# mattmireles/Mamba-ASR

Measured on AMD Instinct MI355X. Metric: encoder audio-frames/sec (ConMamba-large, L=4000), higher is better.
Workload: dtype bf16; 1 GPU; conmamba_large_ctc: encoder forward, 64 utterances x 4000 frames (1000 scan steps) per GPU, random-init weights; global_batch=64, frames_per_utterance=4000, parallelism=utterance shards x1 (no collective in forward), launch=hipGraph replay, streams=2 (join)

## Files before the change

### include/conmamba_hip.h

```cpp
#ifndef CONMAMBA_HIP_H
#define CONMAMBA_HIP_H

#include <stdint.h>

#ifdef __cplusplus
extern "C" {
#endif

#define CM_ABI_VERSION 12

#define CM_OK            0
#define CM_EINVAL       (-1)
#define CM_EUNSUPPORTED (-2)
#define CM_EALIGN       (-3)

typedef enum { CM_F32 = 0, CM_BF16 = 1, CM_F16 = 2 } cm_dtype;

#define CM_SCAN_CHUNK 64

int         cm_abi_version(void);
const char *cm_last_error(void);
int         cm_scan_num_chunks(int seqlen);
#ifdef CM_ABLATE
int         cm_debug_set(int ablation);
// ... 528 lines not shown
    float       *dweight;
    float       *dbias;
    int64_t x_bs, x_ds, y_bs, y_ds, dy_bs, dy_ds, dx_bs, dx_ds;
    void *stream;
} cm_dwconv1d_args;

int cm_dwconv1d_fwd(const cm_dwconv1d_args *args);
int cm_dwconv1d_bwd(const cm_dwconv1d_args *args);

typedef struct cm_dwconv_cl_args {
    int32_t batch, dim, seqlen, ksize, pad_left;
    int32_t io_dtype;
    const void  *x;
    const float *weight;
    const float *bias;
    void        *y;
    const void  *dy;
    void        *dx;
    float       *dweight;
    float       *dbias;
    float       *partial;
    int64_t x_bs, x_ts, y_bs, y_ts, dy_bs, dy_ts, dx_bs, dx_ts;
    void *stream;
    int32_t overwrite;
    int32_t reserved0;
} cm_dwconv_cl_args;

int64_t cm_dwconv_cl_workspace_floats(int32_t batch, int32_t seqlen, int32_t dim);
int cm_dwconv_cl_fwd(const cm_dwconv_cl_args *args);
int cm_dwconv_cl_bwd(const cm_dwconv_cl_args *args);

typedef struct cm_layernorm_args {
    int64_t rows;
    int32_t dim;
    int32_t x_dtype, y_dtype;
    float   eps;
    const void  *x;
    const float *gamma, *beta;
    void  *y;
    float *mean, *rstd;
    const void *dy;
    void  *dx;
    float *dgamma, *dbeta;
    float *workspace;
    void  *stream;
    const float *dres;
    int32_t act;
    float   act_slope;
    const float *chan_mask;
    int32_t mask_rows, mask_c;
} cm_layernorm_args;

int64_t cm_layernorm_bwd_workspace_floats(int64_t rows, int32_t dim);
int cm_layernorm_fwd(const cm_layernorm_args *args);
int cm_layernorm_bwd(const cm_layernorm_args *args);

typedef struct cm_ln_pw_glu_args {
    int32_t rows, dim;
    const float *x;
    const void  *y;
    const float *ln_g, *ln_b;
    const void  *w;
    const float *bias;
    float *x_out;
    void  *out;
    float alpha, eps;
    void *stream;
} cm_ln_pw_glu_args;

int cm_ln_pw_glu(const cm_ln_pw_glu_args *args);

typedef struct cm_ln_pw_glu_mix_args {
    int32_t rows, dim;
    const float *x;
    const float *ln_g, *ln_b;
    const void  *w;
    const float *bias;
    float *x_out;
    void  *out;
    float alpha, eps;
    void *stream;
    const void *ycat;
    const void *proj_w;
    int32_t proj_k;
} cm_ln_pw_glu_mix_args;

int cm_ln_pw_glu_mix(const cm_ln_pw_glu_mix_args *args);

typedef struct cm_cnn_block1_args {
    int32_t batch, T, F, C;
    int32_t io_dtype;
    int32_t pad_out;
    const float *feats;
    const float *weight;
    const float *bias;
    const float *ln_g, *ln_b;
    float eps, slope;
    void *out;
    void *stream;
} cm_cnn_block1_args;

int cm_cnn_block1(const cm_cnn_block1_args *args);

typedef struct cm_cnn_block2_args {
    int32_t batch, T_in, F_in, C_in, C_out;
    int32_t pad_;
    const void  *in;
    const void  *weight;
    const float *bias;
    const float *ln_g, *ln_b;
    float eps, slope;
    void *out;
    void *stream;
} cm_cnn_block2_args;

int cm_cnn_block2(const cm_cnn_block2_args *args);

typedef struct cm_cnn_front_args {
    int32_t batch, T, F, C1, C2;
    int32_t pad_;
    const float *feats;
    const float *w1, *b1, *ln1_g, *ln1_b;
    const void  *w2;
    const float *b2, *ln2_g, *ln2_b;
    float eps1, eps2, slope;
    int32_t pad2_;
    void *out;
    void *stream;
} cm_cnn_front_args;

int cm_cnn_front(const cm_cnn_front_args *args);

typedef struct cm_gemm_args {
    int32_t M, N, K;
    int32_t epilogue;
    const void  *A;  int64_t lda;
    const void  *W;  int64_t ldw;
    const float *bias;
    void        *out; int64_t ldo;
    float       *x;
    float alpha, eps1, eps2;
    int32_t pad_;
    const float *g1, *b1, *g2, *b2;
    void *stream;
} cm_gemm_args;

int cm_gemm_bf16(const cm_gemm_args *args);

int cm_ffn_pack_weights(const void *w , int32_t rows, int32_t cols,
                        void *out , void *stream);

typedef struct cm_ffn_args {
    int32_t rows, dim, hidden;
    int32_t h_dtype;
    const float *x;
    const void  *addend;
    const float *pre_g, *pre_b;
    const void  *w1;
    const float *b1;
    const void  *w2;
    const float *b2;
    const float *n1_g, *n1_b;
    const float *n2_g, *n2_b;
    float       *x_out;
    void        *h_out;
    float add_scale, alpha, pre_eps, n1_eps, n2_eps;
    int32_t proj_dim;
// ... 86 lines not shown
```

### mamba_asr_amd/csrc/ln_pw_glu.hip

```cpp
#include "cm_common.h"


namespace {

typedef __attribute__((ext_vector_type(8))) __bf16 bf16x8;
typedef __attribute__((ext_vector_type(2))) __bf16 bf16x2;
typedef __attribute__((ext_vector_type(4))) float f32x4;
typedef __attribute__((ext_vector_type(2))) float f32x2;
typedef __attribute__((ext_vector_type(4))) unsigned int u32x4;

constexpr int D = 256;
constexpr int TOK = 64;
constexpr int XS = 264;

__device__ __forceinline__ void lds_barrier() { asm volatile("s_waitcnt lgkmcnt(0)\n\ts_barrier" ::: "memory"); }
__device__ __forceinline__ uint32_t pack2(float a, float b) {
    return __builtin_bit_cast(uint32_t, __builtin_convertvector(f32x2{a, b}, bf16x2));
}

constexpr int CK = 128;
constexpr int STAGE = TOK * CK * 2;
static_assert(2 * STAGE <= TOK * XS * 2, "the two ycat stages must fit the token tile they overlay");

struct mix_extra {
    const void *ycat;
    const void *proj_w;
    int32_t proj_k;
};

__device__ __forceinline__ u32x4 raw_rsrc(const void *base, uint32_t bytes) {
    const uint64_t a = reinterpret_cast<uint64_t>(base);
    return u32x4{(uint32_t)a, (uint32_t)(a >> 32) & 0xffffu, bytes, 0x00020000u};
}
__device__ __forceinline__ void dma16(const u32x4 rsrc, uint32_t lds_addr, int voff) {
    uint32_t keep;
    asm volatile("s_mov_b32 %0, m0\n\ts_mov_b32 m0, %1\n\ts_nop 0\n\tbuffer_load_dwordx4 %2, %3, 0 offen lds\n\ts_mov_b32 m0, %0"
                 : "=&s"(keep)
                 : "s"(lds_addr), "v"(voff), "s"(rsrc)
                 : "memory");
}

template <int OCC, int PF, bool MIX>
__global__ __launch_bounds__(256, OCC) void ln_pw_glu_kernel(const cm_ln_pw_glu_args p, const mix_extra mx) {
    __shared__ __attribute__((aligned(16))) uint16_t xn[TOK * XS];
    const int tid = threadIdx.x, lane = tid & 63;
    const int wave = __builtin_amdgcn_readfirstlane(tid >> 6);
    const int l15 = lane & 15, lq = lane >> 4;
    const int t0 = blockIdx.x * TOK, M = p.rows;
    const uint16_t *yv = reinterpret_cast<const uint16_t *>(p.y);

    const __amdgpu_buffer_rsrc_t wr = __builtin_amdgcn_make_buffer_rsrc(const_cast<void *>(p.w), 0, 2 * D * D * 2, 0x00020000);
    const int vl = lane * 16;
    auto wload = [&](int ps, int s, bf16x8(&dst)[2]) {
        const int half = s >> 3, ks = s & 7;
#pragma unroll
        for (int mb = 0; mb < 2; ++mb)
            dst[mb] = __builtin_bit_cast(bf16x8, __builtin_amdgcn_raw_buffer_load_b128(
                                                     wr, vl, (((half * D + wave * 64) / 16 + 2 * ps + mb) * (D / 32) + ks) * 1024, 0));
    };
    bf16x8 wq[PF][2];
    if constexpr (MIX) {
        static_assert(PF == 2, "the projection phase's ring indexing assumes two steps in flight");
        const int K = mx.proj_k, kt = K / 32, nch = K / CK, nstep = 2 * kt;
        const __amdgpu_buffer_rsrc_t pr = __builtin_amdgcn_make_buffer_rsrc(const_cast<void *>(mx.proj_w), 0, D * K * 2, 0x00020000);
        auto pload = [&](int g, bf16x8(&dst)[2]) {
            g = min(g, nstep - 1);
            const int ks = g >> 1, mp = g & 1;
#pragma unroll
            for (int mb = 0; mb < 2; ++mb)
                dst[mb] = __builtin_bit_cast(bf16x8, __builtin_amdgcn_raw_buffer_load_b128(pr, vl, ((wave * 4 + mp * 2 + mb) * kt + ks) * 1024, 0));
        };
        const int vrows = min(TOK, M - t0);
        const u32x4 yr = raw_rsrc(reinterpret_cast<const unsigned char *>(mx.ycat) + (int64_t)t0 * K * 2, (uint32_t)(vrows * K * 2));
        const uint32_t lds0 = (uint32_t)reinterpret_cast<uintptr_t>(&xn[0]);
        int go[4];
#pragma unroll
        for (int i = 0; i < 4; ++i) {
            const int row = 4 * (4 * wave + i) + lq;
            go[i] = row * K * 2 + 16 * (l15 ^ (((row & 3) << 2) | ((row >> 2) & 3)));
        }
        auto request = [&](int c) {
#pragma unroll
            for (int i = 0; i < 4; ++i) dma16(yr, lds0 + (uint32_t)((c & 1) * STAGE + (4 * wave + i) * 1024), go[i] + c * (CK * 2));
        };
        request(0);
#pragma unroll
        for (int s = 0; s < PF; ++s) pload(s, wq[s]);
        f32x4 acc[4][4];
#pragma unroll
        for (int mb = 0; mb < 4; ++mb)
#pragma unroll
            for (int nb = 0; nb < 4; ++nb) acc[mb][nb] = f32x4{0.f, 0.f, 0.f, 0.f};
        const unsigned char *xb = reinterpret_cast<const unsigned char *>(xn);
        const int yrow = l15 * (CK * 2), yswz = ((l15 & 3) << 2) | (l15 >> 2);
        auto read_y = [&](int st, int kk, bf16x8(&bf)[4]) {
            const int off = st * STAGE + yrow + 16 * ((kk * 4 + lq) ^ yswz);
#pragma unroll
            for (int nb = 0; nb < 4; ++nb) bf[nb] = *reinterpret_cast<const bf16x8 *>(xb + off + nb * 16 * (CK * 2));
        };
        for (int c = 0; c < nch; ++c) {
            asm volatile("s_waitcnt vmcnt(0)" ::: "memory");
            lds_barrier();
            if (c + 1 < nch) request(c + 1);
            const int st = c & 1;
            bf16x8 bf[4];
#pragma unroll
            for (int s = 0; s < 8; ++s) {
                const int kk = s >> 1, mp = s & 1;
                if (mp == 0) read_y(st, kk, bf);
#pragma unroll
                for (int mb = 0; mb < 2; ++mb)
#pragma unroll
                    for (int nb = 0; nb < 4; ++nb)
                        acc[mp * 2 + mb][nb] = __builtin_amdgcn_mfma_f32_16x16x32_bf16(wq[s % PF][mb], bf[nb], acc[mp * 2 + mb][nb], 0, 0, 0);
                pload(c * 8 + s + PF, wq[s % PF]);
                __builtin_amdgcn_sched_barrier(0);
            }
        }
        lds_barrier();
#pragma unroll
        for (int mb = 0; mb < 4; ++mb)
#pragma unroll
            for (int nb = 0; nb < 4; ++nb)
                *reinterpret_cast<uint2 *>(xn + (nb * 16 + l15) * XS + wave * 64 + mb * 16 + lq * 4) =
                    uint2{pack2(acc[mb][nb][0], acc[mb][nb][1]), pack2(acc[mb][nb][2], acc[mb][nb][3])};
    }
    if constexpr (MIX) lds_barrier();
    else {
#pragma unroll
        for (int s = 0; s < PF; ++s) wload(0, s, wq[s]);
    }

    {
        float4 v[4][4];
#pragma unroll
        for (int rd = 0; rd < 4; ++rd) {
            const int tok = min(t0 + wave * 16 + rd * 4 + lq, M - 1);
#pragma unroll
            for (int i = 0; i < 4; ++i) {
                const int col = (l15 + 16 * i) * 4;
                float4 x4 = *reinterpret_cast<const float4 *>(p.x + (int64_t)tok * D + col);
                if (MIX || yv) {
                    const uint2 a = MIX ? *reinterpret_cast<const uint2 *>(xn + (wave * 16 + rd * 4 + lq) * XS + col)
                                        : *reinterpret_cast<const uint2 *>(yv + (int64_t)tok * D + col);
                    x4.x = fmaf(p.alpha, cm_bf16_lo(a.x), x4.x);
                    x4.y = fmaf(p.alpha, cm_bf16_hi(a.x), x4.y);
                    x4.z = fmaf(p.alpha, cm_bf16_lo(a.y), x4.z);
                    x4.w = fmaf(p.alpha, cm_bf16_hi(a.y), x4.w);
                }
                v[rd][i] = x4;
            }
        }
#pragma unroll
        for (int rd = 0; rd < 4; ++rd) {
            const int tok = t0 + wave * 16 + rd * 4 + lq;
            if (p.x_out && tok < M) {
#pragma unroll
                for (int i = 0; i < 4; ++i) *reinterpret_cast<float4 *>(p.x_out + (int64_t)tok * D + (l15 + 16 * i) * 4) = v[rd][i];
            }
            float s = 0.f;
#pragma unroll
            for (int i = 0; i < 4; ++i) s += (v[rd][i].x + v[rd][i].y) + (v[rd][i].z + v[rd][i].w);
            const float mean = cm_group_sum<16>(s) * (1.f / D);
            float q = 0.f;
#pragma unroll
            for (int i = 0; i < 4; ++i) {
                v[rd][i].x -= mean; v[rd][i].y -= mean; v[rd][i].z -= mean; v[rd][i].w -= mean;
                q = fmaf(v[rd][i].x, v[rd][i].x, fmaf(v[rd][i].y, v[rd][i].y, fmaf(v[rd][i].z, v[rd][i].z, fmaf(v[rd][i].w, v[rd][i].w, q))));
            }
            const float rstd = rsqrtf(cm_group_sum<16>(q) * (1.f / D) + p.eps);
            uint16_t *dst = xn + (wave * 16 + rd * 4 + lq) * XS;
#pragma unroll
            for (int i = 0; i < 4; ++i) {
                const int col = (l15 + 16 * i) * 4;
                const float4 g = *reinterpret_cast<const float4 *>(p.ln_g + col);
                const float4 b = *reinterpret_cast<const float4 *>(p.ln_b + col);
                uint2 pk;
                pk.x = pack2(fmaf(v[rd][i].x * rstd, g.x, b.x), fmaf(v[rd][i].y * rstd, g.y, b.y));
                pk.y = pack2(fmaf(v[rd][i].z * rstd, g.z, b.z), fmaf(v[rd][i].w * rstd, g.w, b.w));
                *reinterpret_cast<uint2 *>(dst + col) = pk;
            }
        }
    }
    if constexpr (MIX) {
#pragma unroll
        for (int s = 0; s < PF; ++s) wload(0, s, wq[s]);
    }
    lds_barrier();

    const uint16_t *xfrag = xn + l15 * XS + lq * 8;
    auto read_frags = [&](int ks, bf16x8(&bf)[4]) {
#pragma unroll
        for (int nb = 0; nb < 4; ++nb) bf[nb] = *reinterpret_cast<const bf16x8 *>(xfrag + nb * 16 * XS + ks * 32);
    };
    uint16_t *out = reinterpret_cast<uint16_t *>(p.out);
    uint2 held[2][4];
#pragma unroll
    for (int ps = 0; ps < 2; ++ps) {
        f32x4 acc[2][2][4];
#pragma unroll
        for (int h = 0; h < 2; ++h)
#pragma unroll
            for (int mb = 0; mb < 2; ++mb)
#pragma unroll
                for (int nb = 0; nb < 4; ++nb) acc[h][mb][nb] = f32x4{0.f, 0.f, 0.f, 0.f};
        bf16x8 bfa[4], bfb[4];
        read_frags(0, bfa);
#pragma unroll
        for (int s = 0; s < 16; ++s) {
            bf16x8(&cur)[4] = (s & 1) ? bfb : bfa;
            bf16x8(&nxt)[4] = (s & 1) ? bfa : bfb;
            if (s + 1 < 16) read_frags((s + 1) & 7, nxt);
#pragma unroll
            for (int mb = 0; mb < 2; ++mb)
#pragma unroll
                for (int nb = 0; nb < 4; ++nb)
                    acc[s >> 3][mb][nb] = __builtin_amdgcn_mfma_f32_16x16x32_bf16(wq[s % PF][mb], cur[nb], acc[s >> 3][mb][nb], 0, 0, 0);
            if (s + PF < 16) wload(ps, s + PF, wq[s % PF]);
            else if (ps == 0) wload(1, s + PF - 16, wq[s % PF]);
            __builtin_amdgcn_sched_barrier(0);
        }
        const int f0 = wave * 64 + ps * 32 + lq * 4;
#pragma unroll
        for (int mb = 0; mb < 2; ++mb) {
            const float4 ba = *reinterpret_cast<const float4 *>(p.bias + f0 + mb * 16);
            const float4 bg = *reinterpret_cast<const float4 *>(p.bias + D + f0 + mb * 16);
#pragma unroll
            for (int nb = 0; nb < 4; ++nb) {
                const float o0 = (acc[0][mb][nb][0] + ba.x) * cm_sigmoid(acc[1][mb][nb][0] + bg.x);
                const float o1 = (acc[0][mb][nb][1] + ba.y) * cm_sigmoid(acc[1][mb][nb][1] + bg.y);
                const float o2 = (acc[0][mb][nb][2] + ba.z) * cm_sigmoid(acc[1][mb][nb][2] + bg.z);
                const float o3 = (acc[0][mb][nb][3] + ba.w) * cm_sigmoid(acc[1][mb][nb][3] + bg.w);
                if (ps == 0) held[mb][nb] = uint2{pack2(o0, o1), pack2(o2, o3)};
                else {
                    if (mb == 0 && nb == 0) lds_barrier();
                    *reinterpret_cast<uint2 *>(xn + (nb * 16 + l15) * XS + f0 + mb * 16) = uint2{pack2(o0, o1), pack2(o2, o3)};
                    *reinterpret_cast<uint2 *>(xn + (nb * 16 + l15) * XS + f0 - 32 + mb * 16) = held[mb][nb];
                }
            }
        }
    }
    lds_barrier();
#pragma unroll
    for (int i = 0; i < TOK * 32 / 256; ++i) {
        const int idx = tid + 256 * i, row = idx >> 5, chunk = idx & 31;
        const uint4 v = *reinterpret_cast<const uint4 *>(xn + row * XS + chunk * 8);
        if (t0 + row < M) *reinterpret_cast<uint4 *>(out + (int64_t)(t0 + row) * D + chunk * 8) = v;
    }
}

}

int cm_ln_pw_glu144_launch(const cm_ln_pw_glu_args &a);

extern "C" int cm_ln_pw_glu(const cm_ln_pw_glu_args *args) {
    CM_REQUIRE(args != nullptr, CM_EINVAL, "ln_pw_glu: args is NULL");
    const cm_ln_pw_glu_args &a = *args;
    CM_REQUIRE(a.rows > 0 && a.x && a.ln_g && a.ln_b && a.w && a.bias && a.out, CM_EINVAL, "ln_pw_glu: bad sizes or NULL tensor");
    CM_REQUIRE(a.dim == D || a.dim == 144, CM_EUNSUPPORTED, "ln_pw_glu: d_model must be 256 or 144 (got %d)", a.dim);
    CM_REQUIRE(cm_aligned(a.x, 16) && cm_aligned(a.ln_g, 16) && cm_aligned(a.ln_b, 16) && cm_aligned(a.w, 16) && cm_aligned(a.bias, 16) &&
                   cm_aligned(a.out, 16) && (!a.y || cm_aligned(a.y, 8)) && (!a.x_out || cm_aligned(a.x_out, 16)),
               CM_EALIGN, "ln_pw_glu: tensors must be 16-byte aligned (y / out 8)");
    if (a.dim != D) return cm_ln_pw_glu144_launch(a);
    const dim3 grid((a.rows + TOK - 1) / TOK);
    hipStream_t st = reinterpret_cast<hipStream_t>(a.stream);
#ifdef CM_ABLATE
    if (cm_debug_get() == 41) {
        hipLaunchKernelGGL((ln_pw_glu_kernel<3, 4, false>), grid, dim3(256), 0, st, a, mix_extra{});
        return cm_launch_status("cm_ln_pw_glu");
    }
#endif
    hipLaunchKernelGGL((ln_pw_glu_kernel<4, 2, false>), grid, dim3(256), 0, st, a, mix_extra{});
    return cm_launch_status("cm_ln_pw_glu");
}

extern "C" int cm_ln_pw_glu_mix(const cm_ln_pw_glu_mix_args *args) {
    CM_REQUIRE(args != nullptr, CM_EINVAL, "ln_pw_glu_mix: args is NULL");
    const cm_ln_pw_glu_mix_args &m = *args;
    CM_REQUIRE(m.rows > 0 && m.x && m.ln_g && m.ln_b && m.w && m.bias && m.out && m.ycat && m.proj_w, CM_EINVAL,
               "ln_pw_glu_mix: bad sizes or NULL tensor");
    CM_REQUIRE(m.dim == D, CM_EUNSUPPORTED, "ln_pw_glu_mix: d_model must be 256 (got %d)", m.dim);
    CM_REQUIRE(m.proj_k >= CK && m.proj_k % CK == 0 && m.proj_k <= 8192, CM_EUNSUPPORTED,
               "ln_pw_glu_mix: proj_k must be a multiple of 128, at most 8192 (got %d)", m.proj_k);
    CM_REQUIRE(cm_aligned(m.x, 16) && cm_aligned(m.ln_g, 16) && cm_aligned(m.ln_b, 16) && cm_aligned(m.w, 16) && cm_aligned(m.bias, 16) &&
                   cm_aligned(m.out, 16) && cm_aligned(m.ycat, 16) && cm_aligned(m.proj_w, 16) && (!m.x_out || cm_aligned(m.x_out, 16)),
               CM_EALIGN, "ln_pw_glu_mix: tensors must be 16-byte aligned");
    const auto overlap = [](const void *a, int64_t na, const void *b, int64_t nb) {
        const uintptr_t pa = reinterpret_cast<uintptr_t>(a), pb = reinterpret_cast<uintptr_t>(b);
        return a && b && pa < pb + (uintptr_t)nb && pb < pa + (uintptr_t)na;
    };
    const int64_t nx = (int64_t)m.rows * D * 4, no = (int64_t)m.rows * D * 2, ny = (int64_t)m.rows * m.proj_k * 2;
    CM_REQUIRE(!overlap(m.out, no, m.x, nx) && !overlap(m.out, no, m.ycat, ny) && !overlap(m.out, no, m.x_out, nx) &&
                   !overlap(m.x_out, nx, m.ycat, ny) && (m.x_out == m.x || !overlap(m.x_out, nx, m.x, nx)),
               CM_EALIGN, "ln_pw_glu_mix: out / x_out overlap an input (only x_out == x is allowed)");
    cm_ln_pw_glu_args a{};
    a.rows = m.rows, a.dim = m.dim, a.x = m.x, a.y = nullptr, a.ln_g = m.ln_g, a.ln_b = m.ln_b, a.w = m.w, a.bias = m.bias;
    a.x_out = m.x_out, a.out = m.out, a.alpha = m.alpha, a.eps = m.eps, a.stream = m.stream;
    const mix_extra mx{m.ycat, m.proj_w, m.proj_k};
    hipLaunchKernelGGL((ln_pw_glu_kernel<4, 2, true>), dim3((a.rows + TOK - 1) / TOK), dim3(256), 0, reinterpret_cast<hipStream_t>(a.stream), a, mx);
    return cm_launch_status("cm_ln_pw_glu_mix");
}
```

### mamba_asr_amd/fused.py

```python
from __future__ import annotations

import os
from typing import Optional

import torch
import torch.nn.functional as F

from . import ops, weight_cache


class _LayerCache:

    def __init__(self, layer, dtype):
        self.dtype = dtype
        c = lambda t: t.detach().to(dtype).contiguous()
        f = lambda t: None if t is None else t.detach().float().contiguous()
        ffn = lambda m: dict(ln=(f(m[0].weight), f(m[0].bias), m[0].eps), w1=c(m[1].ffn[0].weight), b1=c(m[1].ffn[0].bias),
                             w2=c(m[1].ffn[3].weight), b2=c(m[1].ffn[3].bias), b1f=f(m[1].ffn[0].bias),
                             b2f=f(m[1].ffn[3].bias))
        self.ffn1, self.ffn2 = ffn(layer.ffn_module1), ffn(layer.ffn_module2)
        D = self.ffn1["w1"].shape[1]
        wide = D == 256
        kp = ops._kpad(D)
        d144 = D == 144 and USE_FUSED_D144 and ops.FFN_LAYOUT == 16
        if ops.ffn_supported(D, self.ffn1["w1"].shape[0], dtype) and self.ffn1["w1"].is_cuda and (wide or d144):
            for q in (self.ffn1, self.ffn2):
                q["w1p"] = ops.PackedWeight(q["w1"], ops.FFN_LAYOUT, pad=(q["w1"].shape[0], kp))
                q["w2p"] = ops.PackedWeight(q["w2"], ops.FFN_LAYOUT, pad=(kp, q["w2"].shape[1]))
                if ops.SMALL_FFN_ROWS > 0 and wide:
                    q["w1s"], q["w2s"] = (q["w1p"], q["w2p"]) if ops.FFN_LAYOUT == 32 else (ops.PackedWeight(q["w1"], 32), ops.PackedWeight(q["w2"], 32))
        self.norm1 = (f(layer.norm1.norm.weight), f(layer.norm1.norm.bias), layer.norm1.norm.eps)
        self.norm2 = (f(layer.norm2.norm.weight), f(layer.norm2.norm.bias), layer.norm2.norm.eps)
        m = layer.mamba
        self.d_inner, self.dt_rank, self.d_state = m.d_inner, m.dt_rank, m.d_state
        self.in_proj = c(m.in_proj.weight)
        self.in_packed = None
        if (USE_FFN_INPROJ and dtype == torch.bfloat16 and self.in_proj.is_cuda and self.in_proj.shape[1] == D and (wide or d144)
                and self.in_proj.shape[0] % (256 if wide else 64) == 0 and self.in_proj.shape[0] <= 4096 and m.in_proj.bias is None):
            self.in_packed = ops.PackedWeight(self.in_proj, ops.FFN_LAYOUT, pad=(self.in_proj.shape[0], kp))
            if ops.SMALL_FFN_ROWS > 0 and wide:
                self.in_packed_s = self.in_packed if ops.FFN_LAYOUT == 32 else ops.PackedWeight(self.in_proj, 32)
        self.in_bias = None if m.in_proj.bias is None else c(m.in_proj.bias)
        self.uni = not hasattr(m, "conv1d_b")
        sfxs = ("",) if self.uni else ("", "_b")
        if self.uni:
            self.out_cat = c(m.out_proj.weight)
        else:
            half = 0.5 if m.if_devide_out else 1.0
            self.out_cat = c(torch.cat([m.out_proj.weight, m.out_proj.weight], dim=1) * half)
        self.out_bias = None if m.out_proj.bias is None else c(m.out_proj.bias)
        self.gamma = None if getattr(m, "init_layer_scale", None) is None else f(m.gamma)
        self.dirs = []
        for sfx in sfxs:
            conv, xp, dtp = getattr(m, "conv1d" + sfx), getattr(m, "x_proj" + sfx), getattr(m, "dt_proj" + sfx)
            A_log = getattr(m, "A_b_log" if sfx else "A_log")
            self.dirs.append(dict(conv_w=f(conv.weight).reshape(m.d_inner, -1), conv_b=f(conv.bias), x_proj=c(xp.weight),
                                  dt_proj=c(dtp.weight), dt_proj_f32=c(dtp.weight).float().contiguous(), dt_bias=f(dtp.bias), A=(-torch.exp(A_log.detach().float())).contiguous(),
                                  D=f(getattr(m, "D_b" if sfx else "D"))))
        cm = layer.convolution_module
        xps = [getattr(m, "x_proj" + sfx) for sfx in sfxs]
        self.x_proj_bd = torch.block_diag(*[xp.weight.detach().to(dtype) for xp in xps])
        R, N = self.dt_rank, self.d_state
        self.rows_mode = (R <= 16 or (R <= 32 and dtype == torch.bfloat16)) and N == 16 and m.d_inner % 8 == 0
        if self.rows_mode:
            pad = ops.rows_dt_pad(R)
            self.row_width = pad + 32
            rows = [ops.xproj_rows(xp.weight, R, pad, dtype) for xp in xps]
            self.x_proj_rows = torch.block_diag(*rows)
            self.wx_packed = None
            if dtype == torch.bfloat16 and m.d_inner % 32 == 0 and m.d_inner <= 2048 and rows[0].is_cuda and m.d_conv == 4:
                self.wx_packed = [ops.PackedWeight(r) for r in rows]
            for d_, dtp in zip(self.dirs, [getattr(m, "dt_proj" + sfx) for sfx in sfxs]):
                d_["dt_w16"] = ops.pad_dt_weight(dtp.weight.detach().to(dtype))
        self.cm_ln = (f(cm.layer_norm.weight), f(cm.layer_norm.bias), cm.layer_norm.eps)
        self.pw_w, self.pw_b = c(cm.bottleneck[0].weight.squeeze(-1)), c(cm.bottleneck[0].bias)
        self.pw_bf, self.lin_bf = f(cm.bottleneck[0].bias), f(cm.after_conv[2].bias)
        self.pw_packed = None
        if dtype == torch.bfloat16 and self.pw_w.is_cuda and tuple(self.pw_w.shape) == (2 * D, D) and (wide or d144) and self.pw_bf is not None:
            self.pw_packed = ops.PackedWeight(self.pw_w, pad=(2 * D, kp))
        self.out_packed = None
        if (self.pw_packed is not None and self.out_cat.is_cuda and self.out_cat.shape[0] == 256 and self.out_cat.shape[1] % 128 == 0
                and self.out_cat.shape[1] <= 8192 and self.out_bias is None and self.gamma is None):
            self.out_packed = ops.PackedWeight(self.out_cat)
        self.in_bias_f = None if m.in_proj.bias is None else f(m.in_proj.bias)
        self.out_bias_f = None if m.out_proj.bias is None else f(m.out_proj.bias)
        self.dw_w, self.dw_b = f(cm.conv.weight), f(cm.conv.bias)
        self.dw_wt = self.dw_w.reshape(self.dw_w.shape[0], -1).t().contiguous()
        self.cm_ln2 = (f(cm.after_conv[0].weight), f(cm.after_conv[0].bias), cm.after_conv[0].eps)
        self.lin_w, self.lin_b = c(cm.after_conv[2].weight), c(cm.after_conv[2].bias)
        self.lin_packed = None
        if USE_DWCONV_LIN and dtype == torch.bfloat16 and self.lin_w.is_cuda and tuple(self.lin_w.shape) == (256, 256) and self.lin_bf is not None:
            self.lin_packed = ops.PackedWeight(self.lin_w)
        self.kernel_size, self.causal = cm.kernel_size, bool(cm.causal)

    @property
    def ffn_native(self) -> bool:
        return "w1p" in self.ffn1 and self.ffn2["w1"].shape[0] == self.ffn1["w1"].shape[0]

    @property
    def all_native(self) -> bool:
        return (self.ffn_native and self.rows_mode and self.wx_packed is not None and self.pw_packed is not None
                and self.in_bias is None and self.out_bias is None and self.gamma is None)


def _params_key(dtype, *modules):
    return (dtype,) + tuple((p._version, p.data_ptr()) for m in modules for p in m.parameters())


_LAYER = weight_cache.Kind("_cm_fused_cache", graphs_read=False, build=_LayerCache)


def _cache(layer, dtype) -> _LayerCache:
    return _LAYER.lookup(layer, _params_key(dtype, layer), dtype)


def supports(layer) -> bool:
    from .modules.mamba.bimamba import Mamba as BiMamba, UniMamba
    cm = layer.convolution_module
    act_ok = isinstance(cm.after_conv[1], torch.nn.GELU) and isinstance(layer.ffn_module1[1].ffn[1], torch.nn.GELU)
    mixer_ok = isinstance(layer.mamba, UniMamba) if cm.causal else isinstance(layer.mamba, BiMamba)
    return (mixer_ok and cm.kernel_size == 31 and cm.dilation == 1 and act_ok
            and layer.mamba.d_state == 16 and layer.mamba.d_conv == 4)


def _ffn(x, y_in, p, dtype):
    if dtype == torch.bfloat16:
        h = torch._addmm_activation(p["b1"], y_in, p["w1"].t(), use_gelu=True)
    else:
        h = F.gelu(torch.addmm(p["b1"], y_in, p["w1"].t()))
    return torch.addmm(p["b2"], h, p["w2"].t())


USE_FUSED_D144 = os.environ.get("CM_FUSED_D144", "1") == "1"


USE_FFN_INPROJ = os.environ.get("CM_FFN_INPROJ", "1") == "1"


USE_DWCONV_LIN = os.environ.get("CM_DWCONV_LIN", "1") == "1"


USE_SCAN_ROWS = os.environ.get("CM_SCAN_ROWS", "1") == "1"


USE_CONV_XPROJ = os.environ.get("CM_CONV_XPROJ", "1") == "1"


def _scan_dirs(c: _LayerCache, ucat, ycat, batch, seqlen, xdbl=None):
    E, R, N, nd = c.d_inner, c.dt_rank, c.d_state, len(c.dirs)
    rows, P = batch * seqlen, c.dt_rank + 2 * c.d_state
    if c.rows_mode and (USE_SCAN_ROWS or xdbl is not None):
        if xdbl is None:
            xdbl = (ucat.view(rows, nd * E) @ c.x_proj_rows.t()).view(batch, seqlen, nd * c.row_width)
        RW = c.row_width
        return [dict(u=ucat[:, :, i * E:(i + 1) * E], A=d["A"], D=d["D"], delta_bias=d["dt_bias"], dt_weight=d["dt_w16"],
                     xdbl=xdbl[:, :, RW * i:RW * (i + 1)], out=ycat[:, :, i * E:(i + 1) * E], reverse=bool(i))
                for i, d in enumerate(c.dirs)]
    xdblT = c.x_proj_bd @ ucat.view(rows, nd * E).t()
    feat = ops.alloc_bc(nd * P, batch, seqlen, ucat.device)
    feat.view(nd * P, rows).copy_(xdblT)
    dirs = []
    for i, d in enumerate(c.dirs):
        f = feat[i * P:(i + 1) * P]
        dd = dict(u=ucat[:, :, i * E:(i + 1) * E], A=d["A"], B=f[R:R + N], C=f[R + N:], D=d["D"],
                  delta_bias=d["dt_bias"], out=ycat[:, :, i * E:(i + 1) * E], reverse=bool(i))
        if R <= 16:
            dd.update(dt_low=f[:R], dt_weight=d["dt_proj_f32"])
        else:
            dd["delta"] = (xdblT[i * P:i * P + R].t() @ d["dt_proj"].t()).view(batch, seqlen, E)
        dirs.append(dd)
    return dirs


USE_MIXER_TAIL = os.environ.get("CM_MIXER_TAIL", "1") == "1"


def _out_proj(c: _LayerCache, ycat):
    y = ycat @ c.out_cat.t()
    if c.out_bias is not None:
        y = y + c.out_bias
    if c.gamma is not None:
        y = y * c.gamma.to(y.dtype)
    return y


def mixer_tail(c: _LayerCache, x, ycat):
    if USE_MIXER_TAIL and c.out_packed is not None:
        return ops.ln_pw_glu(x, None, 1.0, c.cm_ln, c.pw_packed, c.pw_bf, ycat=ycat, out_w=c.out_packed)
    return ops.ln_pw_glu(x, _out_proj(c, ycat), 1.0, c.cm_ln, c.pw_packed, c.pw_bf)


def _in_proj(c: _LayerCache, h, out=None):
    xz = torch.mm(h, c.in_proj.t(), out=out)
    return xz if c.in_bias is None else xz.add_(c.in_bias)


def _conv_forms_xdbl(c: _LayerCache) -> bool:
    return USE_CONV_XPROJ and USE_SCAN_ROWS and c.rows_mode and c.wx_packed is not None and c.dtype == torch.bfloat16


def _conv(c: _LayerCache, xz, ucat, xdbl=None, xproj=True, hist=None):
    E = c.d_inner
    if c.uni:
        w0 = (c.dirs[0]["conv_w"], c.dirs[0]["conv_b"])
        if xproj and _conv_forms_xdbl(c):
            x_hist, x_hist_out = hist or (None, None)
            return ops.conv_xproj_uni(xz[:, :, :E], *w0, c.wx_packed[0], out=ucat, xdbl=xdbl, x_hist=x_hist, x_hist_out=x_hist_out)
        assert hist is None
        ops.conv_cl_fwd(xz[:, :, :E], *w0, silu=True, out_f=ucat)
        return None
    w = (c.dirs[0]["conv_w"], c.dirs[0]["conv_b"], c.dirs[1]["conv_w"], c.dirs[1]["conv_b"])
    if xproj and _conv_forms_xdbl(c):
        return ops.conv_xproj(xz[:, :, :E], *w, c.wx_packed[0], c.wx_packed[1], out_f=ucat[:, :, :E], out_b=ucat[:, :, E:], xdbl=xdbl)
    ops.conv_cl_fwd(xz[:, :, :E], *w, True, out_f=ucat[:, :, :E], out_b=ucat[:, :, E:])
    return None


def _scan(c: _LayerCache, xz, ucat, ycat, xdbl, batch, seqlen, state=None):
    dirs = _scan_dirs(c, ucat, ycat, batch, seqlen, xdbl)
    if state is None:
        ops.scan_cl_fwd(dirs, z=xz[:, :, c.d_inner:], delta_softplus=True)
        return
    if len(dirs) != 1 or "xdbl" not in dirs[0]:
        raise NotImplementedError("streaming needs the row-group scan (dt_rank <= 16, or <= 32 in bf16) of a unidirectional mixer")
    ops.scan_cl_fwd([dict(dirs[0], h0=state, h_last=state)], z=xz[:, :, c.d_inner:], delta_softplus=True, time_chunks=1)


def bimamba_fused(c: _LayerCache, h, batch, seqlen):
    xz = _in_proj(c, h).view(batch, seqlen, -1)
    ucat = torch.empty((batch, seqlen, len(c.dirs) * c.d_inner), dtype=xz.dtype, device=xz.device)
    ycat = torch.empty_like(ucat)
    _scan(c, xz, ucat, ycat, _conv(c, xz, ucat), batch, seqlen)
    return _out_proj(c, ycat.view(batch * seqlen, -1))


USE_FUSED_FFN = os.environ.get("CM_FUSED_FFN", "1") == "1"


USE_LN_PW_GLU = os.environ.get("CM_LN_PW_GLU", "1") == "1"


def _ffn_call(x, f, **kw):
    return ops.ffn_fused(x, f["ln"], f["w1p"], f["b1f"], f["w2p"], f["b2f"], alpha=0.5, **kw)


def _ffn_images(c: _LayerCache, small: bool):
    if not (small and "w1s" in c.ffn1):
        return c.ffn1, c.ffn2, c.in_packed
    return (dict(c.ffn1, w1p=c.ffn1["w1s"], w2p=c.ffn1["w2s"]), dict(c.ffn2, w1p=c.ffn2["w1s"], w2p=c.ffn2["w2s"]),
            getattr(c, "in_packed_s", None))


def _head(c: _LayerCache, x, xz, ucat, xdbl=None, small=False, hist=None):
    f1, _, inp = _ffn_images(c, small)
    if c.in_packed is not None:
        _ffn_call(x, f1, norm2=c.norm1, proj_w=inp, proj_out=xz.view(x.shape[0], -1))
    else:
        _in_proj(c, _ffn_call(x, f1, norm2=c.norm1)[1], out=xz.view(x.shape[0], -1))
    return _conv(c, xz, ucat, xdbl, hist=hist)


def _ffn2(c: _LayerCache, x, addend, final_ln=None, f2=None):
    return _ffn_call(x, f2 or c.ffn2, addend=addend, norm1=c.norm2, norm2=final_ln, want_h=final_ln is not None,
                     h_dtype=torch.float32)[1]


def _tail(c: _LayerCache, x, ycat, batch, seqlen, final_ln=None, small=False, hist=None):
    D = x.shape[-1]
    dw = (c.dw_w, c.dw_b, c.cm_ln2[0], c.cm_ln2[1], c.cm_ln2[2])
    kw = dict(causal=True, hist=hist[0], hist_out=hist[1]) if hist is not None else dict(causal=c.causal)
    if USE_LN_PW_GLU and c.pw_packed is not None:
# ... 325 lines not shown
```

### mamba_asr_amd/ops.py

```python
from __future__ import annotations

import ctypes as ct
from typing import Optional, Tuple

import math
import os

import torch

from . import _native as N
from . import weight_cache
from .weight_cache import invalidate_caches

_DT = {torch.float32: N.CM_F32, torch.bfloat16: N.CM_BF16, torch.float16: N.CM_F16}


DETERMINISTIC = os.environ.get("CM_DETERMINISTIC", "1") == "1"


LAUNCH_LOG: Optional[list] = None


def _launch(name: str, fn, args, units: int = 0):
    log = LAUNCH_LOG
# ... 1397 lines not shown
    y = take("y", x2.shape, out_dtype, x.device)
    stats = take("mean", (2, x2.shape[0]), torch.float32, x.device)
    a = _layernorm_args(x2, w, eps, out_dtype)
    a.beta, a.y, a.mean, a.rstd = _ptr(b), _ptr(y), _ptr(stats[0]), _ptr(stats[1])
    _ln_epilogue(a, x2, leaky_slope, chan_mask, mask_rows)
    _launch("cm_layernorm_fwd", N.lib().cm_layernorm_fwd, a, units=x2.shape[0])
    return y.view(x.shape), x2, stats


def layernorm_bwd(dy, x2, stats, weight, eps, need_dx=True, dres=None, bias=None, leaky_slope=None, chan_mask=None, mask_rows=1,
                  bufs=None):
    _dev_check(dy, x2, stats, weight)
    dy2 = dy.reshape(x2.shape)
    if not dy2.is_contiguous():
        dy2 = dy2.contiguous()
    w = weight.detach().float().contiguous()
    take = _bufs(bufs, ("dx", "dgamma", "workspace"), "layernorm_bwd")
    dx = (torch.empty_like(x2) if bufs is None else take("dx", x2.shape, x2.dtype, x2.device)) if need_dx else None
    dgb = take("dgamma", (2, x2.shape[1]), torch.float32, x2.device)
    ws = take("workspace", (N.lib().cm_layernorm_bwd_workspace_floats(x2.shape[0], x2.shape[1]),), torch.float32, x2.device)
    a = _layernorm_args(x2, w, eps, dy2.dtype)
    a.mean, a.rstd, a.dy, a.dx = _ptr(stats[0]), _ptr(stats[1]), _ptr(dy2), _ptr(dx)
    a.dgamma, a.dbeta, a.workspace = _ptr(dgb[0]), _ptr(dgb[1]), _ptr(ws)
    if leaky_slope is not None or chan_mask is not None:
        bb = bias.detach().float().contiguous()
        a.beta = _ptr(bb)
        _ln_epilogue(a, x2, leaky_slope, chan_mask, mask_rows)
    fused_res = dres is not None and need_dx and x2.dtype == torch.float32 and x2.shape[1] <= 1024
    if fused_res:
        _dev_check(dres)
        if dres.dtype != torch.float32 or not dres.is_contiguous() or dres.shape != x2.shape:
            raise RuntimeError("layernorm_bwd: dres must be a contiguous fp32 tensor of x2's shape")
        a.dres = _ptr(dres)
    _launch("cm_layernorm_bwd", N.lib().cm_layernorm_bwd, a, units=x2.shape[0])
    if dres is not None and need_dx and not fused_res:
        dx = dx + dres
    return dx, dgb[0], dgb[1]


class LayerNormFn(torch.autograd.Function):

    @staticmethod
    def forward(ctx, x, weight, bias, eps, low_dtype=None):
        out_dtype = torch.float32 if (x.dtype == torch.float32 or torch.is_autocast_enabled("cuda")) else x.dtype
        if low_dtype is not None:
            out_dtype = low_dtype
        y, x2, stats = layernorm_fwd(x, weight, bias, eps, out_dtype)
        ctx.save_for_backward(x2, stats, weight)
        ctx.eps, ctx.shape = eps, x.shape
        return y

    @staticmethod
    def backward(ctx, dy):
        x2, stats, weight = ctx.saved_tensors
        if dy.dtype not in (torch.float32, torch.bfloat16):
            dy = dy.float()
        dx, dg, db = layernorm_bwd(dy, x2, stats, weight, ctx.eps, need_dx=ctx.needs_input_grad[0])
        return (dx.view(ctx.shape) if dx is not None else None), dg.to(weight.dtype), db.to(weight.dtype), None, None


class LnActDropFn(torch.autograd.Function):

    @staticmethod
    def forward(ctx, x, weight, bias, eps, slope, chan_mask, out_dtype):
        b, t, f, c = x.shape
        x2 = x.reshape(b * t, f * c)
        y, x2s, stats = layernorm_fwd(x2, weight, bias, eps, out_dtype, leaky_slope=slope, chan_mask=chan_mask, mask_rows=t)
        ctx.save_for_backward(x2s, stats, weight, bias, chan_mask if chan_mask is not None else weight.new_empty(0))
        ctx.cfg = (eps, slope, t, chan_mask is not None, x.shape)
        return y.view(x.shape)

    @staticmethod
    def backward(ctx, dy):
        x2, stats, weight, bias, mask = ctx.saved_tensors
        eps, slope, t, has_mask, shape = ctx.cfg
        if dy.dtype not in (torch.float32, torch.bfloat16):
            dy = dy.float()
        dy = dy if dy.is_contiguous() else dy.contiguous()
        dx, dg, db = layernorm_bwd(dy.view(x2.shape[0], -1), x2, stats, weight, eps, need_dx=ctx.needs_input_grad[0], bias=bias, leaky_slope=slope,
                                   chan_mask=mask if has_mask else None, mask_rows=t)
        return (dx.view(shape) if dx is not None else None), dg.to(weight.dtype), db.to(weight.dtype), None, None, None, None


def ln_pw_glu(x, y, alpha, norm, w, bias, x_out=None, ycat=None, out_w=None, out=None):
    _dev_check(x, y, bias, ycat)
    rows, d = x.shape
    if x.dtype != torch.float32 or not x.is_contiguous() or d not in (256, 144):
        raise RuntimeError("ln_pw_glu: x must be a contiguous fp32 (rows, 256) or (rows, 144) tensor")
    if y is not None and (y.dtype != torch.bfloat16 or not y.is_contiguous() or y.shape != x.shape):
        raise RuntimeError("ln_pw_glu: y must be a contiguous bf16 tensor shaped like x")
    if not isinstance(w, PackedWeight) or w.layout != 16 or w.shape != (2 * d, d) or w.padded != (2 * d, _kpad(d)):
        raise RuntimeError("ln_pw_glu: w must be a PackedWeight (16-row tiles) of shape (2D, D), at D = 144 padded to (288, 160)")
    if d != 256 and ycat is not None:
        raise RuntimeError("ln_pw_glu: the projection in front (ycat, out_w) needs d_model 256")
    g_, b_, bs = _f32c(norm[0]), _f32c(norm[1]), _f32c(bias)
    xo = x if x_out is None else x_out
    out = _out_rows(out, (rows, d), torch.bfloat16, x.device, "ln_pw_glu: out")
    if (ycat is None) != (out_w is None) or (ycat is not None and y is not None):
        raise RuntimeError("ln_pw_glu: give either y, or ycat together with out_w")
    if ycat is not None:
        if ycat.dtype != torch.bfloat16 or not ycat.is_contiguous() or ycat.dim() != 2 or ycat.shape[0] != rows:
            raise RuntimeError("ln_pw_glu: ycat must be a contiguous bf16 (rows, K) tensor")
        if not isinstance(out_w, PackedWeight) or out_w.layout != 16 or out_w.shape != (256, ycat.shape[1]):
            raise RuntimeError("ln_pw_glu: out_w must be a PackedWeight (16-row tiles) of shape (256, K)")
        m = N.LnPwGluMixArgs()
        m.rows, m.dim, m.x, m.ln_g, m.ln_b, m.w, m.bias = rows, d, _ptr(x), _ptr(g_), _ptr(b_), _ptr(w.data), _ptr(bs)
        m.x_out, m.out, m.alpha, m.eps, m.stream = _ptr(xo), _ptr(out), float(alpha), float(norm[2]), _stream()
        m.ycat, m.proj_w, m.proj_k = _ptr(ycat), _ptr(out_w.data), ycat.shape[1]
        _launch("cm_ln_pw_glu", N.lib().cm_ln_pw_glu_mix, m, units=rows)
        return out
    a = N.LnPwGluArgs()
    a.rows, a.dim, a.x, a.y, a.ln_g, a.ln_b, a.w, a.bias = rows, d, _ptr(x), _ptr(y), _ptr(g_), _ptr(b_), _ptr(w.data), _ptr(bs)
    a.x_out, a.out, a.alpha, a.eps, a.stream = _ptr(xo), _ptr(out), float(alpha), float(norm[2]), _stream()
    _launch("cm_ln_pw_glu", N.lib().cm_ln_pw_glu, a, units=rows)
    return out


def glu_dwconv_ln_gelu(inp, weight, bias, ln_weight, ln_bias, eps=1e-5, weight_t=None, glu_done=False, lin_w=None, lin_b=None,
                       variant: int = 0, causal: bool = False, hist=None, hist_out=None, out=None):
    _dev_check(inp, weight, bias, ln_weight, ln_bias, hist, hist_out)
    if (hist is not None or hist_out is not None) and not causal:
        raise RuntimeError("glu_dwconv_ln_gelu: hist / hist_out belong to the causal form")
    if not inp.is_contiguous():
        inp = inp.contiguous()
    b, l, d2 = inp.shape
    d = d2 if glu_done else d2 // 2
    w = _f32c(weight).reshape(d, -1)
    bs, g, bt = _f32c(bias), _f32c(ln_weight), _f32c(ln_bias)
    out = _out_rows(out, (b, l, d), inp.dtype, inp.device, "glu_dwconv_ln_gelu: out")
    a = N.GluDwconvCausalArgs() if causal else N.GluDwconvArgs()
    if causal:
        hs = (b, w.shape[1] - 1, d)
        a.hist, a.hist_out = _ptr(_hist_rows(hist, hs, inp.dtype, "glu_dwconv_ln_gelu: hist")), _ptr(_hist_rows(hist_out, hs, inp.dtype, "glu_dwconv_ln_gelu: hist_out"))
    a.batch, a.seqlen, a.dim, a.ksize, a.io_dtype, a.glu_done = b, l, d, w.shape[1], _DT[inp.dtype], int(bool(glu_done))
    a.in_, a.weight, a.bias, a.ln_g, a.ln_b, a.eps, a.out = _ptr(inp), _ptr(w), _ptr(bs), _ptr(g), _ptr(bt), float(eps), _ptr(out)
    wt = w.t().contiguous() if weight_t is None else weight_t
    if wt.dtype != torch.float32 or wt.shape != (w.shape[1], d) or not wt.is_contiguous():
        raise RuntimeError("glu_dwconv_ln_gelu: weight_t must be a contiguous fp32 (k, dim) tensor")
    a.weight_t = _ptr(wt)
    if lin_w is not None:
        if not isinstance(lin_w, PackedWeight) or lin_w.shape != (d, d) or lin_b is None:
            raise RuntimeError("glu_dwconv_ln_gelu: lin_w must be a PackedWeight of shape (dim, dim), with lin_b")
        lb = _f32c(lin_b)
        a.lin_w, a.lin_b = _ptr(lin_w.data), _ptr(lb)
    a.stream, a.variant = _stream(), int(variant)
    if causal:
        _launch("cm_glu_dwconv_ln_gelu_causal", N.lib().cm_glu_dwconv_ln_gelu_causal, a, units=b * l)
    else:
        _launch("cm_glu_dwconv_ln_gelu", N.lib().cm_glu_dwconv_ln_gelu, a, units=b * l)
    return out


def cnn_block1(feats, weight, bias, ln_weight, ln_bias, eps=1e-5, slope=0.01, out_dtype=torch.bfloat16, pad_out=1):
    _dev_check(feats, weight, bias, ln_weight, ln_bias)
    feats = feats.float().contiguous()
    b, t, f = feats.shape
    w, bs, g, bt = _f32c(weight), _f32c(bias), _f32c(ln_weight), _f32c(ln_bias)
    cch = w.shape[0]
    t1, f1 = (t + 1) // 2, (f + 1) // 2
    out = torch.empty((b, t1 + 2 * pad_out, f1 + 2 * pad_out, cch), dtype=out_dtype, device=feats.device)
    a = N.CnnBlock1Args()
    a.batch, a.T, a.F, a.C, a.io_dtype, a.pad_out = b, t, f, cch, _DT[out_dtype], pad_out
    a.feats, a.weight, a.bias, a.ln_g, a.ln_b, a.eps, a.slope, a.out = (_ptr(feats), _ptr(w), _ptr(bs), _ptr(g), _ptr(bt),
                                                                          float(eps), float(slope), _ptr(out))
    a.stream = _stream()
    _launch("cm_cnn_block1", N.lib().cm_cnn_block1, a, units=b * t)
    return out


def cnn_front_supported(feats, w1, w2_ohwi) -> bool:
    return (feats.shape[-1] == 80 and tuple(w1.shape) == (64, 1, 3, 3) and tuple(w2_ohwi.shape) == (32, 3, 3, 64)
            and w2_ohwi.dtype == torch.bfloat16 and feats.shape[1] >= 5)


def cnn_front(feats, w1, b1, ln1_w, ln1_b, eps1, w2_ohwi, b2, ln2_w, ln2_b, eps2, slope=0.01):
    _dev_check(feats, w1, b1, ln1_w, ln1_b, w2_ohwi, b2, ln2_w, ln2_b)
    feats = feats.float().contiguous()
    if not cnn_front_supported(feats, w1, w2_ohwi) or not w2_ohwi.is_contiguous():
        raise RuntimeError("cnn_front: needs 80 bins, a (64, 1, 3, 3) first conv and a contiguous bf16 (32, 3, 3, 64) second conv")
    b, t, f = feats.shape
    t1 = (t + 1) // 2
    t2 = (t1 - 1) // 2 + 1
    w1f, b1f, g1, bt1 = _f32c(w1), _f32c(b1), _f32c(ln1_w).reshape(-1), _f32c(ln1_b).reshape(-1)
    b2f, g2, bt2 = _f32c(b2), _f32c(ln2_w).reshape(-1), _f32c(ln2_b).reshape(-1)
    if g1.numel() != 40 * 64 or g2.numel() != 20 * 32:
        raise RuntimeError("cnn_front: LayerNorm parameters must have 40*64 and 20*32 elements")
    out = torch.empty((b, t2, 640), dtype=torch.bfloat16, device=feats.device)
    a = N.CnnFrontArgs()
    a.batch, a.T, a.F, a.C1, a.C2 = b, t, f, 64, 32
    a.feats, a.w1, a.b1, a.ln1_g, a.ln1_b = _ptr(feats), _ptr(w1f), _ptr(b1f), _ptr(g1), _ptr(bt1)
    a.w2, a.b2, a.ln2_g, a.ln2_b = _ptr(w2_ohwi), _ptr(b2f), _ptr(g2), _ptr(bt2)
# ... 305 lines not shown
```

Before: 21.80 million audio-frames/s.

## Reuse each out-proj weight fragment across both scan directions in fused mixer tail

The fused out-projection inside ln_pw_glu no longer multiplies against a concatenated [W, W] weight. It now loads the single (256, K) weight once per K step and applies it to the forward and backward ycat halves from two LDS sub-stages. This halves the projection-weight bytes streamed per tile and drops the doubled weight copy. In exchange the chunk depth, DMA addressing and swizzle change, the kernel gains a DIRS template parameter, and the C ABI struct gets a new proj_dirs field.

```diff
diff --git a/include/conmamba_hip.h b/include/conmamba_hip.h
--- a/include/conmamba_hip.h
+++ b/include/conmamba_hip.h
@@ -634,7 +634,7 @@
     void *stream;
     const void *ycat;
     const void *proj_w;
-    int32_t proj_k;
+    int32_t proj_k, proj_dirs;
 } cm_ln_pw_glu_mix_args;
 
 int cm_ln_pw_glu_mix(const cm_ln_pw_glu_mix_args *args);
diff --git a/mamba_asr_amd/csrc/ln_pw_glu.hip b/mamba_asr_amd/csrc/ln_pw_glu.hip
--- a/mamba_asr_amd/csrc/ln_pw_glu.hip
+++ b/mamba_asr_amd/csrc/ln_pw_glu.hip
@@ -18,14 +18,15 @@
     return __builtin_bit_cast(uint32_t, __builtin_convertvector(f32x2{a, b}, bf16x2));
 }
 
-constexpr int CK = 128;
-constexpr int STAGE = TOK * CK * 2;
+constexpr int CK = 64;
+constexpr int SUB = TOK * CK * 2;
+constexpr int STAGE = 2 * SUB;
 static_assert(2 * STAGE <= TOK * XS * 2, "the two ycat stages must fit the token tile they overlay");
 
 struct mix_extra {
     const void *ycat;
     const void *proj_w;
-    int32_t proj_k;
+    int32_t kw;
 };
 
 __device__ __forceinline__ u32x4 raw_rsrc(const void *base, uint32_t bytes) {
@@ -40,8 +41,9 @@
                  : "memory");
 }
 
-template <int OCC, int PF, bool MIX>
+template <int OCC, int PF, int DIRS>
 __global__ __launch_bounds__(256, OCC) void ln_pw_glu_kernel(const cm_ln_pw_glu_args p, const mix_extra mx) {
+    constexpr bool MIX = DIRS > 0;
     __shared__ __attribute__((aligned(16))) uint16_t xn[TOK * XS];
     const int tid = threadIdx.x, lane = tid & 63;
     const int wave = __builtin_amdgcn_readfirstlane(tid >> 6);
@@ -61,7 +63,8 @@
     bf16x8 wq[PF][2];
     if constexpr (MIX) {
         static_assert(PF == 2, "the projection phase's ring indexing assumes two steps in flight");
-        const int K = mx.proj_k, kt = K / 32, nch = K / CK, nstep = 2 * kt;
+        constexpr int KT = 4 / DIRS;
+        const int K = mx.kw, kt = K / 32, nch = kt / KT, nstep = 2 * kt, RB = DIRS * K * 2;
         const __amdgpu_buffer_rsrc_t pr = __builtin_amdgcn_make_buffer_rsrc(const_cast<void *>(mx.proj_w), 0, D * K * 2, 0x00020000);
         auto pload = [&](int g, bf16x8(&dst)[2]) {
             g = min(g, nstep - 1);
@@ -71,17 +74,14 @@
                 dst[mb] = __builtin_bit_cast(bf16x8, __builtin_amdgcn_raw_buffer_load_b128(pr, vl, ((wave * 4 + mp * 2 + mb) * kt + ks) * 1024, 0));
         };
         const int vrows = min(TOK, M - t0);
-        const u32x4 yr = raw_rsrc(reinterpret_cast<const unsigned char *>(mx.ycat) + (int64_t)t0 * K * 2, (uint32_t)(vrows * K * 2));
+        const u32x4 yr = raw_rsrc(reinterpret_cast<const unsigned char *>(mx.ycat) + (int64_t)t0 * RB, (uint32_t)(vrows * RB));
         const uint32_t lds0 = (uint32_t)reinterpret_cast<uintptr_t>(&xn[0]);
-        int go[4];
-#pragma unroll
-        for (int i = 0; i < 4; ++i) {
-            const int row = 4 * (4 * wave + i) + lq;
-            go[i] = row * K * 2 + 16 * (l15 ^ (((row & 3) << 2) | ((row >> 2) & 3)));
-        }
+        const int row0 = 32 * (wave & 1) + (lane >> 3);
+        const int go0 = row0 * RB + (wave >> 1) * (DIRS == 2 ? K * 2 : CK * 2) + 16 * ((lane & 7) ^ ((row0 >> 1) & 7));
         auto request = [&](int c) {
 #pragma unroll
-            for (int i = 0; i < 4; ++i) dma16(yr, lds0 + (uint32_t)((c & 1) * STAGE + (4 * wave + i) * 1024), go[i] + c * (CK * 2));
+            for (int i = 0; i < 4; ++i)
+                dma16(yr, lds0 + (uint32_t)((c & 1) * STAGE + (4 * wave + i) * 1024), (go0 ^ ((i & 1) << 6)) + (8 * i * RB + c * (KT * 64)));
         };
         request(0);
 #pragma unroll
@@ -92,9 +92,9 @@
 #pragma unroll
             for (int nb = 0; nb < 4; ++nb) acc[mb][nb] = f32x4{0.f, 0.f, 0.f, 0.f};
         const unsigned char *xb = reinterpret_cast<const unsigned char *>(xn);
-        const int yrow = l15 * (CK * 2), yswz = ((l15 & 3) << 2) | (l15 >> 2);
-        auto read_y = [&](int st, int kk, bf16x8(&bf)[4]) {
-            const int off = st * STAGE + yrow + 16 * ((kk * 4 + lq) ^ yswz);
+        const int yrow = l15 * (CK * 2), yswz = (l15 >> 1) & 7;
+        auto read_y = [&](int st, int j, int kk, bf16x8(&bf)[4]) {
+            const int off = st * STAGE + j * SUB + yrow + 16 * ((kk * 4 + lq) ^ yswz);
 #pragma unroll
             for (int nb = 0; nb < 4; ++nb) bf[nb] = *reinterpret_cast<const bf16x8 *>(xb + off + nb * 16 * (CK * 2));
         };
@@ -105,16 +105,21 @@
             const int st = c & 1;
             bf16x8 bf[4];
 #pragma unroll
-            for (int s = 0; s < 8; ++s) {
-                const int kk = s >> 1, mp = s & 1;
-                if (mp == 0) read_y(st, kk, bf);
-#pragma unroll
-                for (int mb = 0; mb < 2; ++mb)
-#pragma unroll
-                    for (int nb = 0; nb < 4; ++nb)
-                        acc[mp * 2 + mb][nb] = __builtin_amdgcn_mfma_f32_16x16x32_bf16(wq[s % PF][mb], bf[nb], acc[mp * 2 + mb][nb], 0, 0, 0);
-                pload(c * 8 + s + PF, wq[s % PF]);
-                __builtin_amdgcn_sched_barrier(0);
+            for (int t = 0; t < KT; ++t) {
+#pragma unroll
+                for (int d = 0; d < DIRS; ++d) {
+                    read_y(st, DIRS == 2 ? d : t >> 1, DIRS == 2 ? t : t & 1, bf);
+#pragma unroll
+                    for (int mp = 0; mp < 2; ++mp) {
+#pragma unroll
+                        for (int mb = 0; mb < 2; ++mb)
+#pragma unroll
+                            for (int nb = 0; nb < 4; ++nb)
+                                acc[mp * 2 + mb][nb] = __builtin_amdgcn_mfma_f32_16x16x32_bf16(wq[mp][mb], bf[nb], acc[mp * 2 + mb][nb], 0, 0, 0);
+                        if (d == DIRS - 1) pload(2 * (c * KT + t) + mp + PF, wq[mp]);
+                        __builtin_amdgcn_sched_barrier(0);
+                    }
+                }
             }
         }
         lds_barrier();
@@ -241,9 +246,10 @@
         }
     }
     lds_barrier();
+    const int tid2 = wave * 64 + (int)__builtin_amdgcn_mbcnt_hi(~0u, __builtin_amdgcn_mbcnt_lo(~0u, 0u));
 #pragma unroll
     for (int i = 0; i < TOK * 32 / 256; ++i) {
-        const int idx = tid + 256 * i, row = idx >> 5, chunk = idx & 31;
+        const int idx = tid2 + 256 * i, row = idx >> 5, chunk = idx & 31;
         const uint4 v = *reinterpret_cast<const uint4 *>(xn + row * XS + chunk * 8);
         if (t0 + row < M) *reinterpret_cast<uint4 *>(out + (int64_t)(t0 + row) * D + chunk * 8) = v;
     }
@@ -266,11 +272,11 @@
     hipStream_t st = reinterpret_cast<hipStream_t>(a.stream);
 #ifdef CM_ABLATE
     if (cm_debug_get() == 41) {
-        hipLaunchKernelGGL((ln_pw_glu_kernel<3, 4, false>), grid, dim3(256), 0, st, a, mix_extra{});
+        hipLaunchKernelGGL((ln_pw_glu_kernel<3, 4, 0>), grid, dim3(256), 0, st, a, mix_extra{});
         return cm_launch_status("cm_ln_pw_glu");
     }
 #endif
-    hipLaunchKernelGGL((ln_pw_glu_kernel<4, 2, false>), grid, dim3(256), 0, st, a, mix_extra{});
+    hipLaunchKernelGGL((ln_pw_glu_kernel<4, 2, 0>), grid, dim3(256), 0, st, a, mix_extra{});
     return cm_launch_status("cm_ln_pw_glu");
 }
 
@@ -280,7 +286,7 @@
     CM_REQUIRE(m.rows > 0 && m.x && m.ln_g && m.ln_b && m.w && m.bias && m.out && m.ycat && m.proj_w, CM_EINVAL,
                "ln_pw_glu_mix: bad sizes or NULL tensor");
     CM_REQUIRE(m.dim == D, CM_EUNSUPPORTED, "ln_pw_glu_mix: d_model must be 256 (got %d)", m.dim);
-    CM_REQUIRE(m.proj_k >= CK && m.proj_k % CK == 0 && m.proj_k <= 8192, CM_EUNSUPPORTED,
+    CM_REQUIRE(m.proj_k >= 128 && m.proj_k % 128 == 0 && m.proj_k <= 8192, CM_EUNSUPPORTED,
                "ln_pw_glu_mix: proj_k must be a multiple of 128, at most 8192 (got %d)", m.proj_k);
     CM_REQUIRE(cm_aligned(m.x, 16) && cm_aligned(m.ln_g, 16) && cm_aligned(m.ln_b, 16) && cm_aligned(m.w, 16) && cm_aligned(m.bias, 16) &&
                    cm_aligned(m.out, 16) && cm_aligned(m.ycat, 16) && cm_aligned(m.proj_w, 16) && (!m.x_out || cm_aligned(m.x_out, 16)),
@@ -296,7 +302,13 @@
     cm_ln_pw_glu_args a{};
     a.rows = m.rows, a.dim = m.dim, a.x = m.x, a.y = nullptr, a.ln_g = m.ln_g, a.ln_b = m.ln_b, a.w = m.w, a.bias = m.bias;
     a.x_out = m.x_out, a.out = m.out, a.alpha = m.alpha, a.eps = m.eps, a.stream = m.stream;
-    const mix_extra mx{m.ycat, m.proj_w, m.proj_k};
-    hipLaunchKernelGGL((ln_pw_glu_kernel<4, 2, true>), dim3((a.rows + TOK - 1) / TOK), dim3(256), 0, reinterpret_cast<hipStream_t>(a.stream), a, mx);
+    CM_REQUIRE(m.proj_dirs == 1 || m.proj_dirs == 2, CM_EINVAL, "ln_pw_glu_mix: proj_dirs must be 1 or 2 (got %d)", m.proj_dirs);
+    CM_REQUIRE(m.proj_k % (128 * m.proj_dirs) == 0, CM_EUNSUPPORTED,
+               "ln_pw_glu_mix: proj_k must be proj_dirs x the weight's K, K a multiple of 128 (got %d for %d blocks)", m.proj_k, m.proj_dirs);
+    const mix_extra mx{m.ycat, m.proj_w, m.proj_k / m.proj_dirs};
+    const dim3 grid((a.rows + TOK - 1) / TOK);
+    hipStream_t st = reinterpret_cast<hipStream_t>(a.stream);
+    if (m.proj_dirs == 2) hipLaunchKernelGGL((ln_pw_glu_kernel<4, 2, 2>), grid, dim3(256), 0, st, a, mx);
+    else hipLaunchKernelGGL((ln_pw_glu_kernel<4, 2, 1>), grid, dim3(256), 0, st, a, mx);
     return cm_launch_status("cm_ln_pw_glu_mix");
 }
diff --git a/mamba_asr_amd/fused.py b/mamba_asr_amd/fused.py
--- a/mamba_asr_amd/fused.py
+++ b/mamba_asr_amd/fused.py
@@ -43,11 +43,8 @@
         self.in_bias = None if m.in_proj.bias is None else c(m.in_proj.bias)
         self.uni = not hasattr(m, "conv1d_b")
         sfxs = ("",) if self.uni else ("", "_b")
-        if self.uni:
-            self.out_cat = c(m.out_proj.weight)
-        else:
-            half = 0.5 if m.if_devide_out else 1.0
-            self.out_cat = c(torch.cat([m.out_proj.weight, m.out_proj.weight], dim=1) * half)
+        self.out_w = c(m.out_proj.weight * (1.0 if self.uni or not m.if_devide_out else 0.5))
+        self._out_cat = None
         self.out_bias = None if m.out_proj.bias is None else c(m.out_proj.bias)
         self.gamma = None if getattr(m, "init_layer_scale", None) is None else f(m.gamma)
         self.dirs = []
@@ -79,9 +76,9 @@
         if dtype == torch.bfloat16 and self.pw_w.is_cuda and tuple(self.pw_w.shape) == (2 * D, D) and (wide or d144) and self.pw_bf is not None:
             self.pw_packed = ops.PackedWeight(self.pw_w, pad=(2 * D, kp))
         self.out_packed = None
-        if (self.pw_packed is not None and self.out_cat.is_cuda and self.out_cat.shape[0] == 256 and self.out_cat.shape[1] % 128 == 0
-                and self.out_cat.shape[1] <= 8192 and self.out_bias is None and self.gamma is None):
-            self.out_packed = ops.PackedWeight(self.out_cat)
+        if (self.pw_packed is not None and self.out_w.is_cuda and self.out_w.shape[0] == 256 and self.out_w.shape[1] % 128 == 0
+                and len(sfxs) * self.out_w.shape[1] <= 8192 and self.out_bias is None and self.gamma is None):
+            self.out_packed = ops.PackedWeight(self.out_w)
         self.in_bias_f = None if m.in_proj.bias is None else f(m.in_proj.bias)
         self.out_bias_f = None if m.out_proj.bias is None else f(m.out_proj.bias)
         self.dw_w, self.dw_b = f(cm.conv.weight), f(cm.conv.bias)
@@ -92,6 +89,12 @@
         if USE_DWCONV_LIN and dtype == torch.bfloat16 and self.lin_w.is_cuda and tuple(self.lin_w.shape) == (256, 256) and self.lin_bf is not None:
             self.lin_packed = ops.PackedWeight(self.lin_w)
         self.kernel_size, self.causal = cm.kernel_size, bool(cm.causal)
+
+    @property
+    def out_cat(self):
+        if self._out_cat is None:
+            self._out_cat = self.out_w if self.uni else torch.cat([self.out_w, self.out_w], dim=1)
+        return self._out_cat
 
     @property
     def ffn_native(self) -> bool:
@@ -186,7 +189,7 @@
 
 def mixer_tail(c: _LayerCache, x, ycat):
     if USE_MIXER_TAIL and c.out_packed is not None:
-        return ops.ln_pw_glu(x, None, 1.0, c.cm_ln, c.pw_packed, c.pw_bf, ycat=ycat, out_w=c.out_packed)
+        return ops.ln_pw_glu(x, None, 1.0, c.cm_ln, c.pw_packed, c.pw_bf, ycat=ycat, out_w=c.out_packed, dirs=len(c.dirs))
     return ops.ln_pw_glu(x, _out_proj(c, ycat), 1.0, c.cm_ln, c.pw_packed, c.pw_bf)
 
 
diff --git a/mamba_asr_amd/ops.py b/mamba_asr_amd/ops.py
--- a/mamba_asr_amd/ops.py
+++ b/mamba_asr_amd/ops.py
@@ -1503,7 +1503,7 @@
         return (dx.view(shape) if dx is not None else None), dg.to(weight.dtype), db.to(weight.dtype), None, None, None, None
 
 
-def ln_pw_glu(x, y, alpha, norm, w, bias, x_out=None, ycat=None, out_w=None, out=None):
+def ln_pw_glu(x, y, alpha, norm, w, bias, x_out=None, ycat=None, out_w=None, out=None, dirs=1):
     _dev_check(x, y, bias, ycat)
     rows, d = x.shape
     if x.dtype != torch.float32 or not x.is_contiguous() or d not in (256, 144):
@@ -1522,12 +1522,12 @@
     if ycat is not None:
         if ycat.dtype != torch.bfloat16 or not ycat.is_contiguous() or ycat.dim() != 2 or ycat.shape[0] != rows:
             raise RuntimeError("ln_pw_glu: ycat must be a contiguous bf16 (rows, K) tensor")
-        if not isinstance(out_w, PackedWeight) or out_w.layout != 16 or out_w.shape != (256, ycat.shape[1]):
-            raise RuntimeError("ln_pw_glu: out_w must be a PackedWeight (16-row tiles) of shape (256, K)")
+        if dirs not in (1, 2) or not isinstance(out_w, PackedWeight) or out_w.layout != 16 or (256, dirs * out_w.shape[1]) != (out_w.shape[0], ycat.shape[1]):
+            raise RuntimeError("ln_pw_glu: dirs must be 1 or 2 and out_w a PackedWeight (16-row tiles) of shape (256, K), ycat dirs * K wide")
         m = N.LnPwGluMixArgs()
         m.rows, m.dim, m.x, m.ln_g, m.ln_b, m.w, m.bias = rows, d, _ptr(x), _ptr(g_), _ptr(b_), _ptr(w.data), _ptr(bs)
         m.x_out, m.out, m.alpha, m.eps, m.stream = _ptr(xo), _ptr(out), float(alpha), float(norm[2]), _stream()
-        m.ycat, m.proj_w, m.proj_k = _ptr(ycat), _ptr(out_w.data), ycat.shape[1]
+        m.ycat, m.proj_w, m.proj_k, m.proj_dirs = _ptr(ycat), _ptr(out_w.data), ycat.shape[1], dirs
         _launch("cm_ln_pw_glu", N.lib().cm_ln_pw_glu_mix, m, units=rows)
         return out
     a = N.LnPwGluArgs()
```

Result: no change. 21.93 million audio-frames/s, median of 6 (+0.6%).
